# FluidInference/FluidAudio

Hardware: NVIDIA H100
Metric: audio-hours/s (higher is better)
Workload: dtype f32

## Files before the change

fluidaudio_b200/csrc/mel_core.cuh:

```cuda
#pragma once

#include "fa_common.cuh"
#include <math.h>
#include <stdint.h>

namespace fa {
namespace mel {

constexpr int kNfft = 512;
constexpr int kHalf = 256;
constexpr int kBins = 257;
constexpr int kFftPad = 304;
constexpr int kTileFrames = 16;
constexpr int kPairStride = 524;
FA_HD int pow_pos(int bin) { return bin ^ ((bin >> 4) & 3); }

struct alignas(8) cpx {
    float x, y;
};

struct alignas(8) f32x2 {
    float a, b;
};

#if defined(__CUDA_ARCH__)
__device__ __forceinline__ float2 as_f2(f32x2 v) { return make_float2(v.a, v.b); }
__device__ __forceinline__ f32x2 as_v(float2 v) {
    f32x2 r;
    r.a = v.x;
    r.b = v.y;
    return r;
}
#endif

FA_HD double vadd(double x, double y) { return x + y; }
FA_HD double vsub(double x, double y) { return x - y; }
FA_HD double vneg(double x) { return -x; }
FA_HD double vmul_s(double x, double s) { return x * s; }
FA_HD double vfma_s(double a, double s, double c) { return a * s + c; }
FA_HD double vfnma_s(double a, double s, double c) { return c - a * s; }

FA_HD f32x2 vneg(f32x2 x) {
    f32x2 r;
    r.a = -x.a;
    r.b = -x.b;
    return r;
}
#if defined(__CUDA_ARCH__)
__device__ __forceinline__ f32x2 vadd(f32x2 x, f32x2 y) { return as_v(fadd2_rn(as_f2(x), as_f2(y))); }
__device__ __forceinline__ f32x2 vsub(f32x2 x, f32x2 y) { return as_v(fadd2_rn(as_f2(x), as_f2(vneg(y)))); }
__device__ __forceinline__ f32x2 vmul_s(f32x2 x, float s) { return as_v(fmul2_rn(as_f2(x), make_float2(s, s))); }
__device__ __forceinline__ f32x2 vfma_s(f32x2 a, float s, f32x2 c) {
    return as_v(ffma2_rn(as_f2(a), make_float2(s, s), as_f2(c)));
}
__device__ __forceinline__ f32x2 vfnma_s(f32x2 a, float s, f32x2 c) {
    return as_v(ffma2_rn(as_f2(vneg(a)), make_float2(s, s), as_f2(c)));
}
#else
inline f32x2 vadd(f32x2 x, f32x2 y) { return f32x2{x.a + y.a, x.b + y.b}; }
inline f32x2 vsub(f32x2 x, f32x2 y) { return f32x2{x.a - y.a, x.b - y.b}; }
inline f32x2 vmul_s(f32x2 x, float s) { return f32x2{x.a * s, x.b * s}; }
inline f32x2 vfma_s(f32x2 a, float s, f32x2 c) { return f32x2{fmaf(a.a, s, c.a), fmaf(a.b, s, c.b)}; }
inline f32x2 vfnma_s(f32x2 a, float s, f32x2 c) { return f32x2{fmaf(-a.a, s, c.a), fmaf(-a.b, s, c.b)}; }
#endif

template <typename V>
struct vtraits;
template <>
struct vtraits<double> {
    typedef double scalar;
    static constexpr int kFrames = 1;
};
template <>
struct vtraits<f32x2> {
    typedef float scalar;
    static constexpr int kFrames = 2;
};

template <typename V>
struct alignas(16) cpxv {
    V x, y;
};
typedef cpxv<double> cpxd;
struct cpxs {
    float x, y;
};

struct LaneCommon {
    float win[16];
    uint32_t in_win;
    int a1, a2, k0;
    int k0s, kc0s;
};
template <typename V>
struct LaneTables;
template <>
struct LaneTables<double> : LaneCommon {
    cpxd w256;
    cpxd w32;
    cpxd wk0;
};
template <>
struct LaneTables<f32x2> : LaneCommon {
    cpxs tw1[8];
    cpxs tw2[8];
    cpxs wk[4];
};

FA_HD void lane_butterflies(int l, int &c1, int &c2) {
    if (l >= 8) {
        c1 = l;
        c2 = 8 * (8 - (l >> 3)) + (7 - (l & 7));
    } else if (l >= 4) {
        c1 = 32 + (l - 4);
        c2 = 39 - (l - 4);
    } else if (l >= 1) {
        c1 = l;
        c2 = 8 - l;
    } else {
        c1 = 0;
        c2 = 4;
    }
}

FA_HD cpxd unit_root(int k, int n) {
    const double a = -6.283185307179586476925286766559 * (double)k / (double)n;
    cpxd r;
    r.x = cos(a);
    r.y = sin(a);
    return r;
}
FA_HD cpxs unit_root_f(int k, int n) {
    const cpxd d = unit_root(k, n);
    cpxs r;
    r.x = (float)d.x;
    r.y = (float)d.y;
    return r;
}

FA_HD void load_lane_common(int l, const float *win_tab, const uint8_t *in_tab, LaneCommon &T) {
    T.in_win = 0;
#pragma unroll
    for (int r = 0; r < 8; ++r) {
        const int j = 2 * (l + 32 * r);
        T.win[2 * r] = win_tab[j];
        T.win[2 * r + 1] = win_tab[j + 1];
        if (in_tab[j]) T.in_win |= 1u << (2 * r);
        if (in_tab[j + 1]) T.in_win |= 1u << (2 * r + 1);
    }
    int c1, c2;
    lane_butterflies(l, c1, c2);
    T.a1 = 9 * (c1 >> 3) + (c1 & 7);
    T.a2 = 9 * (c2 >> 3) + (c2 & 7);
    T.k0 = (c1 >> 3) + 8 * (c1 & 7);
    T.k0s = pow_pos(T.k0);
    T.kc0s = pow_pos(kHalf - T.k0);
}
FA_HD void load_lane_tables(int l, const float *win_tab, const uint8_t *in_tab, LaneTables<double> &T) {
    load_lane_common(l, win_tab, in_tab, T);
    T.w256 = unit_root(l, 256);
    T.w32 = unit_root(l & 3, 32);
    T.wk0 = unit_root(T.k0, 512);
}
FA_HD void load_lane_tables(int l, const float *win_tab, const uint8_t *in_tab, LaneTables<f32x2> &T) {
    load_lane_common(l, win_tab, in_tab, T);
#pragma unroll
    for (int q = 0; q < 8; ++q) {
        T.tw1[q] = unit_root_f((l * q) & 255, 256);
        T.tw2[q] = unit_root_f(((l & 3) * q) & 31, 32);
    }
#pragma unroll
    for (int k2 = 0; k2 < 4; ++k2) T.wk[k2] = unit_root_f(T.k0 + 64 * k2, 512);
}

FA_HD cpxd cmul(cpxd a, cpxd b) {
    cpxd r;
    r.x = a.x * b.x - a.y * b.y;
    r.y = a.x * b.y + a.y * b.x;
    return r;
}

template <typename V>
FA_HD void dft4(V &r0, V &i0, V &r1, V &i1, V &r2, V &i2, V &r3, V &i3) {
    const V ar = vadd(r0, r2), ai = vadd(i0, i2);
    const V br = vsub(r0, r2), bi = vsub(i0, i2);
    const V cr = vadd(r1, r3), ci = vadd(i1, i3);
    const V dr = vsub(r1, r3), di = vsub(i1, i3);
    r0 = vadd(ar, cr);
    i0 = vadd(ai, ci);
    r2 = vsub(ar, cr);
    i2 = vsub(ai, ci);
    r1 = vadd(br, di);
    i1 = vsub(bi, dr);
    r3 = vsub(br, di);
    i3 = vadd(bi, dr);
}

template <typename V>
FA_HD void dft8(V (&re)[8], V (&im)[8]) {
    typedef typename vtraits<V>::scalar S;
    const S kS = (S)0.70710678118654752440;
    V er0 = vadd(re[0], re[4]), ei0 = vadd(im[0], im[4]);
    V er1 = vadd(re[1], re[5]), ei1 = vadd(im[1], im[5]);
    V er2 = vadd(re[2], re[6]), ei2 = vadd(im[2], im[6]);
    V er3 = vadd(re[3], re[7]), ei3 = vadd(im[3], im[7]);
    V or0 = vsub(re[0], re[4]), oi0 = vsub(im[0], im[4]);
    const V xr1 = vsub(re[1], re[5]), xi1 = vsub(im[1], im[5]);
    const V xr2 = vsub(re[2], re[6]), xi2 = vsub(im[2], im[6]);
    const V xr3 = vsub(re[3], re[7]), xi3 = vsub(im[3], im[7]);
    V or1 = vmul_s(vadd(xr1, xi1), kS), oi1 = vmul_s(vsub(xi1, xr1), kS);
    V or2 = xi2, oi2 = vneg(xr2);
    V or3 = vmul_s(vsub(xi3, xr3), kS), oi3 = vmul_s(vadd(xr3, xi3), (S)(-kS));
    dft4(er0, ei0, er1, ei1, er2, ei2, er3, ei3);
    dft4(or0, oi0, or1, oi1, or2, oi2, or3, oi3);
    re[0] = er0; im[0] = ei0;
    re[2] = er1; im[2] = ei1;
    re[4] = er2; im[4] = ei2;
    re[6] = er3; im[6] = ei3;
    re[1] = or0; im[1] = oi0;
    re[3] = or1; im[3] = oi1;
    re[5] = or2; im[5] = oi2;
    re[7] = or3; im[7] = oi3;
}

template <typename Emit>
FA_HD void twiddle_emit(double (&re)[8], double (&im)[8], cpxd root, Emit emit) {
    cpxd p[8];
    p[1] = root;
    p[2] = cmul(root, root);
    p[3] = cmul(p[2], root);
    p[4] = cmul(p[2], p[2]);
    p[5] = cmul(p[4], root);
    p[6] = cmul(p[4], p[2]);
    p[7] = cmul(p[4], p[3]);
    cpxd v;
    v.x = re[0];
    v.y = im[0];
    emit(0, v);
#pragma unroll
    for (int q = 1; q < 8; ++q) {
        v.x = re[q] * p[q].x - im[q] * p[q].y;
        v.y = re[q] * p[q].y + im[q] * p[q].x;
        emit(q, v);
    }
}
template <typename Emit>
FA_HD void twiddle_emit(f32x2 (&re)[8], f32x2 (&im)[8], const cpxs (&tw)[8], Emit emit) {
    cpxv<f32x2> v;
    v.x = re[0];
    v.y = im[0];
    emit(0, v);
#pragma unroll
    for (int q = 1; q < 8; ++q) {
        v.x = vfnma_s(im[q], tw[q].y, vmul_s(re[q], tw[q].x));
        v.y = vfma_s(im[q], tw[q].x, vmul_s(re[q], tw[q].y));
        emit(q, v);
    }
}
FA_HD void twiddle_pass1(int l, double (&re)[8], double (&im)[8], const LaneTables<double> &T, cpxd *buf) {
    twiddle_emit(re, im, T.w256, [&](int q, cpxd v) { buf[l + 36 * q] = v; });
}
FA_HD void twiddle_pass1(int l, f32x2 (&re)[8], f32x2 (&im)[8], const LaneTables<f32x2> &T, cpxv<f32x2> *buf) {
    twiddle_emit(re, im, T.tw1, [&](int q, cpxv<f32x2> v) { buf[l + 36 * q] = v; });
}
FA_HD void twiddle_pass2(int base, double (&re)[8], double (&im)[8], const LaneTables<double> &T, cpxd *buf) {
    twiddle_emit(re, im, T.w32, [&](int q2, cpxd v) { buf[base + q2] = v; });
}
FA_HD void twiddle_pass2(int base, f32x2 (&re)[8], f32x2 (&im)[8], const LaneTables<f32x2> &T, cpxv<f32x2> *buf) {
    twiddle_emit(re, im, T.tw2, [&](int q2, cpxv<f32x2> v) { buf[base + q2] = v; });
}

FA_HD void widen(float a, float b, float, float, double &re, double &im) {
    re = (double)a;
    im = (double)b;
}
FA_HD void widen(float a, float b, float a2, float b2, f32x2 &re, f32x2 &im) {
    re.a = a;
    re.b = a2;
    im.a = b;
    im.b = b2;
}

template <bool kMidFull, typename V>
FA_HD void pass1(int l, const float *pf, int hop, const LaneTables<V> &T, cpxv<V> *buf) {
    V re[8], im[8];
#pragma unroll
    for (int r = 0; r < 8; ++r) {
        const int j = 2 * (l + 32 * r);
#if defined(__CUDA_ARCH__)
        const float2 v = *reinterpret_cast<const float2 *>(pf + j);
        float2 u = v;
        if (vtraits<V>::kFrames == 2) u = *reinterpret_cast<const float2 *>(pf + hop + j);
#else
        const cpx v = *reinterpret_cast<const cpx *>(pf + j);
        cpx u = v;
        if (vtraits<V>::kFrames == 2) u = *reinterpret_cast<const cpx *>(pf + hop + j);
#endif
        float a = T.win[2 * r] * v.x, b = T.win[2 * r + 1] * v.y;
        float a2 = T.win[2 * r] * u.x, b2 = T.win[2 * r + 1] * u.y;
        if (!kMidFull || r == 0 || r == 7) {
            const bool ia = (T.in_win >> (2 * r)) & 1u, ib = (T.in_win >> (2 * r + 1)) & 1u;
            a = ia ? a : 0.0f;
            b = ib ? b : 0.0f;
            a2 = ia ? a2 : 0.0f;
            b2 = ib ? b2 : 0.0f;
        }
        widen(a, b, a2, b2, re[r], im[r]);
    }
    dft8(re, im);
    twiddle_pass1(l, re, im, T, buf);
}

template <typename V>
FA_HD void pass2_load(int l, const cpxv<V> *buf, V (&re)[8], V (&im)[8]) {
    const int base = 36 * (l >> 2) + (l & 3);
#pragma unroll
    for (int r = 0; r < 8; ++r) {
        const cpxv<V> v = buf[base + 4 * r];
        re[r] = v.x;
        im[r] = v.y;
    }
}
template <typename V>
FA_HD void pass2_store(int l, const LaneTables<V> &T, V (&re)[8], V (&im)[8], cpxv<V> *buf) {
    dft8(re, im);
    const int base = 74 * (l & 3) + 9 * (l >> 2);
    twiddle_pass2(base, re, im, T, buf);
}

FA_HD void pair_power(double zbx, double zby, double zcx, double zcy, double wx, double wy, float *prow, int ib, int ic) {
    const double sr = zbx + zcx, si = zby - zcy;
    const double dr = zby + zcy, di = zcx - zbx;
    const double tr = wx * dr - wy * di, ti = wx * di + wy * dr;
    const float xr = (float)(sr + tr), xi = (float)(si + ti);
    const float yr = (float)(sr - tr), yi = (float)(si - ti);
#if defined(__CUDA_ARCH__)
    prow[2 * ib] = __fadd_rn(__fmul_rn(xr, xr), __fmul_rn(xi, xi));
    prow[2 * ic] = __fadd_rn(__fmul_rn(yr, yr), __fmul_rn(yi, yi));
#else
    const float a = xr * xr, b = xi * xi, c = yr * yr, d = yi * yi;
    prow[2 * ib] = a + b;
    prow[2 * ic] = c + d;
#endif
}
FA_HD void pair_power(f32x2 zbx, f32x2 zby, f32x2 zcx, f32x2 zcy, float wx, float wy, float *prow, int ib, int ic) {
    const f32x2 sr = vadd(zbx, zcx), si = vsub(zby, zcy);
    const f32x2 dr = vadd(zby, zcy), di = vsub(zcx, zbx);
    const f32x2 tr = vfnma_s(di, wy, vmul_s(dr, wx)), ti = vfma_s(dr, wy, vmul_s(di, wx));
    const f32x2 xr = vadd(sr, tr), xi = vadd(si, ti);
    const f32x2 yr = vsub(sr, tr), yi = vsub(si, ti);
#if defined(__CUDA_ARCH__)
    const float2 pb = ffma2_rn(as_f2(xr), as_f2(xr), fmul2_rn(as_f2(xi), as_f2(xi)));
    const float2 pc = ffma2_rn(as_f2(yr), as_f2(yr), fmul2_rn(as_f2(yi), as_f2(yi)));
    *reinterpret_cast<float2 *>(prow + 2 * ib) = pb;
    *reinterpret_cast<float2 *>(prow + 2 * ic) = pc;
#else
    prow[2 * ib] = fmaf(xr.a, xr.a, xi.a * xi.a);
    prow[2 * ic] = fmaf(yr.a, yr.a, yi.a * yi.a);
    prow[2 * ib + 1] = fmaf(xr.b, xr.b, xi.b * xi.b);
    prow[2 * ic + 1] = fmaf(yr.b, yr.b, yi.b * yi.b);
#endif
}

FA_HD void recombination_roots(const LaneTables<double> &T, double (&wx)[4], double (&wy)[4]) {
    const double hh = 0.70710678118654752440;
    wx[0] = T.wk0.x;
    wy[0] = T.wk0.y;
    wx[1] = hh * (wx[0] + wy[0]);
    wy[1] = hh * (wy[0] - wx[0]);
    wx[2] = wy[0];
    wy[2] = -wx[0];
    wx[3] = wy[1];
    wy[3] = -wx[1];
}
FA_HD void recombination_roots(const LaneTables<f32x2> &T, float (&wx)[4], float (&wy)[4]) {
#pragma unroll
    for (int k = 0; k < 4; ++k) {
        wx[k] = T.wk[k].x;
        wy[k] = T.wk[k].y;
    }
}

template <typename V>
FA_HD void pass3_post(int l, const cpxv<V> *buf, const LaneTables<V> &T, float *prow) {
    typedef typename vtraits<V>::scalar S;
    V ar[4], ai[4], br[4], bi[4];
#pragma unroll
    for (int h = 0; h < 4; ++h) {
        const cpxv<V> u = buf[T.a1 + 74 * h], v = buf[T.a2 + 74 * h];
        ar[h] = u.x;
        ai[h] = u.y;
        br[h] = v.x;
        bi[h] = v.y;
    }
    dft4(ar[0], ai[0], ar[1], ai[1], ar[2], ai[2], ar[3], ai[3]);
    dft4(br[0], bi[0], br[1], bi[1], br[2], bi[2], br[3], bi[3]);
    const bool z = l == 0;
    const S c1 = (S)0.92387953251128675613, s1 = (S)0.38268343236508977173;
    S wx[4], wy[4];
    recombination_roots(T, wx, wy);
    pair_power(ar[0], ai[0], z ? ar[0] : br[3], z ? ai[0] : bi[3], wx[0], wy[0], prow, T.k0s, T.kc0s);
    pair_power(ar[1], ai[1], z ? ar[3] : br[2], z ? ai[3] : bi[2], wx[1], wy[1], prow, T.k0s + 64, T.kc0s - 64);
    pair_power(ar[2], ai[2], z ? ar[2] : br[1], z ? ai[2] : bi[1], wx[2], wy[2], prow, T.k0s + 128, T.kc0s - 128);
    const int b3 = z ? pow_pos(32) : T.k0s + 192, c3 = z ? pow_pos(224) : T.kc0s - 192;
    pair_power(z ? br[0] : ar[3], z ? bi[0] : ai[3], z ? br[3] : br[0], z ? bi[3] : bi[0], z ? c1 : wx[3],
               z ? (S)(-s1) : wy[3], prow, b3, c3);
    if (z) {
        pair_power(br[1], bi[1], br[2], bi[2], s1, (S)(-c1), prow, pow_pos(96), pow_pos(160));
    }
}

FA_HD float mel_dot(const float *prow, const float *w, int lo, int hi) {
    float acc = 0.0f;
    const float *p = prow + lo;
    const int n = hi - lo;
    for (int b = 0; b < n; ++b) {
        const float t = w[b] * p[b];
        acc = acc + t;
    }
    return acc;
}
#if defined(__CUDACC__)
__device__ __forceinline__ float2 mel_dot_pairs(const float4 *p4, const float4 *w4, int nq) {
    float2 acc = make_float2(0.0f, 0.0f);
#pragma unroll 1
    for (int b = 0; b < nq; ++b) {
        const float4 x01 = p4[2 * b], x23 = p4[2 * b + 1], c = w4[b];
        acc = ffma2_rn(make_float2(x01.x, x01.y), make_float2(c.x, c.x), acc);
        acc = ffma2_rn(make_float2(x01.z, x01.w), make_float2(c.y, c.y), acc);
        acc = ffma2_rn(make_float2(x23.x, x23.y), make_float2(c.z, c.z), acc);
        acc = ffma2_rn(make_float2(x23.z, x23.w), make_float2(c.w, c.w), acc);
    }
    return acc;
}
__device__ __forceinline__ float mel_dot_quads(const float4 *p4, const float4 *w4, int nq) {
    float acc = 0.0f;
#pragma unroll 1
    for (int b = 0; b < nq; ++b) {
        const float4 x = p4[b], c = w4[b];
        acc = fmaf(c.x, x.x, acc);
        acc = fmaf(c.y, x.y, acc);
        acc = fmaf(c.z, x.z, acc);
        acc = fmaf(c.w, x.w, acc);
    }
    return acc;
}
#endif

FA_HD float log_value(float v, float floor_, int clamped, int normal_floor = 0) {
    const float x = clamped ? (floor_ >= v ? floor_ : v) : v + floor_;
#if defined(__CUDA_ARCH__)
    float l;
    if (normal_floor) asm("lg2.approx.ftz.f32 %0, %1;" : "=f"(l) : "f"(x));
    else l = __log2f(x);
    return l * 0.693147180559945309417f;
#else
    (void)normal_floor;
    return logf(x);
#endif
}

FA_HD float preemph_first(float x0, float last, float a) {
#if defined(__CUDA_ARCH__)
    return __fsub_rn(x0, __fmul_rn(a, last));
#else
    const float t = a * last;
    return x0 - t;
#endif
}
FA_HD float preemph_rest(float x, float xprev, float a) { return fmaf(xprev, -a, x); }

}
}
```

fluidaudio_b200/csrc/mel_kernels.cu:

```cuda
#include "mel_core.cuh"
#include "mel_plan.h"

#include <cuda_runtime.h>
#include <algorithm>
#include <cmath>
#include <cstdio>
#include <cstdlib>
#include <cstring>
#include <limits>
#include <vector>

namespace fa {
namespace mel {

__device__ __forceinline__ uint32_t smem_u32(const void *p) { return (uint32_t)__cvta_generic_to_shared(p); }

__device__ __forceinline__ void mbar_init(uint64_t *bar, uint32_t count) {
    asm volatile("mbarrier.init.shared::cta.b64 [%0], %1;" ::"r"(smem_u32(bar)), "r"(count));
}
__device__ __forceinline__ void mbar_expect_tx(uint64_t *bar, uint32_t bytes) {
    asm volatile("mbarrier.arrive.expect_tx.shared::cta.b64 _, [%0], %1;" ::"r"(smem_u32(bar)), "r"(bytes) : "memory");
}
__device__ __forceinline__ void mbar_arrive(uint64_t *bar) {
    asm volatile("mbarrier.arrive.shared::cta.b64 _, [%0];" ::"r"(smem_u32(bar)) : "memory");
}
__device__ __forceinline__ bool mbar_try_wait(uint64_t *bar, uint32_t parity) {
    uint32_t ok;
    asm volatile(
        "{\n\t"
        ".reg .pred p;\n\t"
        "mbarrier.try_wait.parity.shared::cta.b64 p, [%1], %2;\n\t"
        "selp.u32 %0, 1, 0, p;\n\t"
        "}"
        : "=r"(ok)
        : "r"(smem_u32(bar)), "r"(parity)
        : "memory");
    return ok != 0;
}
__device__ __forceinline__ void mbar_wait(uint64_t *bar, uint32_t parity) {
    while (!mbar_try_wait(bar, parity)) {
    }
}
__device__ __forceinline__ void bulk_g2s(void *dst, const void *src, uint32_t bytes, uint64_t *bar) {
    asm volatile("cp.async.bulk.shared::cluster.global.mbarrier::complete_tx::bytes [%0], [%1], %2, [%3];" ::"r"(
                     smem_u32(dst)),
                 "l"(src), "r"(bytes), "r"(smem_u32(bar))
                 : "memory");
}
__device__ __forceinline__ void fence_proxy_async() { asm volatile("fence.proxy.async.shared::cta;" ::: "memory"); }

struct TileGeom {
    int unit;
    long long f0;
    int nf;
    long long a0;
    long long base;
    long long gs, ge;
};

__device__ __forceinline__ const MelUnit &unit_at(const MelLaunch &P, int idx) { return P.inline_unit ? P.unit0 : P.units[idx]; }

__device__ __forceinline__ TileGeom tile_geom(const MelLaunch &P, int tile) {
    int lo = 0, hi = P.inline_unit ? 0 : P.num_units - 1;
    while (lo < hi) {
        const int mid = (lo + hi + 1) >> 1;
        if (P.units[mid].tile_begin <= tile) lo = mid; else hi = mid - 1;
    }
    const MelUnit &u = P.inline_unit ? P.unit0 : P.units[lo];
    TileGeom g;
    g.unit = lo;
    g.f0 = u.frame_begin + (long long)kTileFrames * (tile - u.tile_begin);
    const long long rem = u.frame_begin + u.frame_count - g.f0;
    g.nf = rem < kTileFrames ? (int)rem : kTileFrames;
    g.a0 = g.f0 * P.hop - P.pad;
    const long long need0 = g.a0 - 1;
    g.base = (need0 >= 0) ? (need0 & ~3LL) : -(((-need0) + 3) & ~3LL);
    long long ge = (g.a0 + P.pt_len + 3) & ~3LL;
    const long long n4 = u.n & ~3LL;
    if (ge > n4) ge = n4;
    g.gs = g.base < 0 ? 0 : g.base;
    g.ge = ge;
    if (!P.use_tma) g.ge = g.gs;
    return g;
}

struct TileInfo {
    TileGeom g;
    long long audio_off, n, out_off, out_stride;
    float last;
    int pad_;
};
__device__ __forceinline__ void make_tile_info(const MelLaunch &P, int tile, TileInfo &ti) {
    ti.g = tile_geom(P, tile);
    const MelUnit &u = unit_at(P, ti.g.unit);
    ti.audio_off = u.audio_off;
    ti.n = u.n;
    ti.out_off = u.out_off;
    ti.out_stride = u.out_stride;
    ti.last = u.last;
}

template <int kWarps, typename V, int kLayout>
__global__ void __launch_bounds__(kWarps * 32, 2) mel512_kernel(const MelLaunch P) {
    constexpr int kF = vtraits<V>::kFrames;
    extern __shared__ __align__(128) unsigned char smem[];
    float *raw0 = reinterpret_cast<float *>(smem);
    float *raw1 = raw0 + P.raw_cap;
    float *ptile = raw1 + P.raw_cap;
    cpxv<V> *fftbuf = reinterpret_cast<cpxv<V> *>(ptile + P.pt_cap);
    float *power = reinterpret_cast<float *>(fftbuf + kWarps * kFftPad);
    float *otile = power + (kTileFrames / 2) * kPairStride;
    const int ot_stride = P.ot_stride;
    float *fbw = otile + kTileFrames * ot_stride;
    int4 *fbmeta = reinterpret_cast<int4 *>(fbw + P.fb_cap);
    uint64_t *bars = reinterpret_cast<uint64_t *>(fbmeta + P.n_slots);
    TileInfo *tinfo = reinterpret_cast<TileInfo *>(bars + 2);

    const int tid = threadIdx.x, lane = tid & 31, warp = tid >> 5;

    if (tid == 0) {
        mbar_init(&bars[0], 1);
        mbar_init(&bars[1], 1);
        asm volatile("fence.mbarrier_init.release.cluster;" ::: "memory");
    }
    for (int i = tid; i < P.fb_nnz; i += kWarps * 32) fbw[i] = P.fb_w[i];
    for (int i = tid; i < P.n_slots; i += kWarps * 32) fbmeta[i] = P.fb_slots[i];
    for (int i = tid; i < (kTileFrames / 2) * kPairStride; i += kWarps * 32) power[i] = 0.0f;
    const LaneTables<V> T = reinterpret_cast<const LaneTables<V> *>(P.lane_tab)[lane];
    __syncthreads();

    cpxv<V> *buf = fftbuf + warp * kFftPad;

    auto issue = [&](int tile, int buf, TileInfo &slot) {
        make_tile_info(P, tile, slot);
        const TileGeom &g = slot.g;
        float *dst = buf ? raw1 : raw0;
        if (g.ge > g.gs) {
            const uint32_t bytes = (uint32_t)((g.ge - g.gs) * 4);
            mbar_expect_tx(&bars[buf], bytes);
            bulk_g2s(dst + (g.gs - g.base), P.audio + slot.audio_off + g.gs, bytes, &bars[buf]);
        } else {
            mbar_arrive(&bars[buf]);
        }
    };

    auto preemphasize = [&](const TileInfo &u, const float *raw) {
        const TileGeom &g = u.g;
        const float a = P.preemph;
        const bool interior = g.a0 >= 1 && g.a0 - 1 >= g.gs && g.a0 + P.pt_len <= g.ge && g.a0 + P.pt_len <= u.n;
        if (interior) {
            const float *src = raw + (g.a0 - g.base);
            if (((g.a0 - g.base) & 3) == 0 && (P.pt_len & 3) == 0) {
                const float4 *s4 = reinterpret_cast<const float4 *>(src);
                float4 *d4 = reinterpret_cast<float4 *>(ptile);
                for (int q = tid; q < (P.pt_len >> 2); q += kWarps * 32) {
                    const float4 x = s4[q];
                    float4 y = x;
                    const float prev = src[4 * q - 1];
                    if (a != 0.0f) {
                        y.x = preemph_rest(x.x, prev, a);
                        y.y = preemph_rest(x.y, x.x, a);
                        y.z = preemph_rest(x.z, x.y, a);
                        y.w = preemph_rest(x.w, x.z, a);
                    }
                    d4[q] = y;
                }
            } else if (a == 0.0f) {
                for (int t = tid; t < P.pt_len; t += kWarps * 32) ptile[t] = src[t];
            } else {
                for (int t = tid; t < P.pt_len; t += kWarps * 32) ptile[t] = preemph_rest(src[t], src[t - 1], a);
            }
        } else {
            const float *gaudio = P.audio + u.audio_off;
            auto sample = [&](long long i) -> float {
                if (i >= g.gs && i < g.ge) return raw[i - g.base];
                if (i < 0) return u.last;
                return __ldg(gaudio + i);
            };
            for (int t = tid; t < P.pt_len; t += kWarps * 32) {
                const long long i = g.a0 + t;
                float v = 0.0f;
                if (i >= 0 && i < u.n) {
                    const float x = sample(i);
                    if (a == 0.0f) v = x;
                    else if (i == 0) v = preemph_first(x, u.last, a);
                    else v = preemph_rest(x, sample(i - 1), a);
                }
                ptile[t] = v;
            }
        }
    };
    auto copy_out = [&](float *dst, int total) {
        if (P.out_vec4) {
            float4 *d4 = reinterpret_cast<float4 *>(dst);
            for (int q = tid; q < (total >> 2); q += kWarps * 32) {
                const int e = 4 * q;
                const int row = (int)__umulhi((unsigned)e, P.inv_n_mels);
                d4[q] = *reinterpret_cast<const float4 *>(otile + e + 4 * row);
            }
        } else {
            const int row_pad = ot_stride - P.n_mels;
            for (int idx = tid; idx < total; idx += kWarps * 32) {
                const int fi = P.n_mels == 1 ? idx : (int)__umulhi((unsigned)idx, P.inv_n_mels);
                dst[idx] = otile[idx + fi * row_pad];
            }
        }
    };

    const int first = blockIdx.x, stride = gridDim.x;
    if (first >= P.total_tiles) return;
    if (tid == 0) {
        issue(first, 0, tinfo[0]);
        if (first + stride < P.total_tiles) issue(first + stride, 1, tinfo[1]);
    }
    __syncthreads();
    mbar_wait(&bars[0], 0);
    preemphasize(tinfo[0], raw0);
    __syncthreads();
    float *pending_dst = nullptr;
    int pending_total = 0;
    int it = 0, slot = 0;
    for (int tile = first; tile < P.total_tiles; tile += stride, ++it, slot = slot == 2 ? 0 : slot + 1) {
        const TileInfo &u = tinfo[slot];
        const int nf = u.g.nf;

        if (pending_dst) copy_out(pending_dst, pending_total);
        for (int fi = warp * kF; fi < nf; fi += kWarps * kF) {
            const float *pf = ptile + fi * P.hop;
            V re[8], im[8];
            if (P.mid_full) pass1<true>(lane, pf, P.hop, T, buf); else pass1<false>(lane, pf, P.hop, T, buf);
            __syncwarp();
            pass2_load(lane, buf, re, im);
            __syncwarp();
            pass2_store(lane, T, re, im, buf);
            __syncwarp();
            pass3_post(lane, buf, T, power + (fi >> 1) * kPairStride + (fi & 1));
            __syncwarp();
        }
        __syncthreads();

        const int next = tile + stride;
        const int slot1 = slot == 2 ? 0 : slot + 1, slot2 = slot1 == 2 ? 0 : slot1 + 1;
        if (tid == 0 && next + stride < P.total_tiles) {
            fence_proxy_async();
            issue(next + stride, it & 1, tinfo[slot2]);
        }
        {
            constexpr int kPairs = kTileFrames / 2, kGroup = 32 / kPairs;
            const int pl = lane % kPairs, mg = lane / kPairs;
            const float *prow = power + pl * kPairStride;
            float *orow = otile + (2 * pl) * ot_stride;
            float *gout = kLayout == 1 ? P.out + u.out_off + u.g.f0 + 2 * pl : nullptr;
            for (int slot = warp * kGroup + mg; slot < P.n_slots; slot += kWarps * kGroup) {
                const int4 md = fbmeta[slot];
                const float2 a2 = mel_dot_pairs(reinterpret_cast<const float4 *>(prow + 2 * md.x),
                                                reinterpret_cast<const float4 *>(fbw + md.z), md.y);
                const float v0 = log_value(a2.x, P.log_floor, P.log_clamped, P.log_normal),
                            v1 = log_value(a2.y, P.log_floor, P.log_clamped, P.log_normal);
                const int m = md.w;
                if (m < 0) continue;
                if (kLayout == 0) {
                    orow[m] = v0;
                    orow[ot_stride + m] = v1;
                } else {
                    float *g = gout + (long long)m * u.out_stride;
                    if (2 * pl < nf) g[0] = v0;
                    if (2 * pl + 1 < nf) g[1] = v1;
                }
            }
        }
        if (kLayout == 0) {
            pending_dst = P.out + u.out_off + u.g.f0 * P.n_mels;
            pending_total = nf * P.n_mels;
        }
        if (next < P.total_tiles) {
            const int nb = (it + 1) & 1;
            mbar_wait(&bars[nb], (uint32_t)((it + 1) >> 1) & 1u);
            preemphasize(tinfo[slot1], nb ? raw1 : raw0);
        }
        __syncthreads();
    }
    if (pending_dst) copy_out(pending_dst, pending_total);
}


struct GenericParams {
    int n_fft, log2n, bins, prow;
    const cpxd *tw;
    int warps;
};

__global__ void __launch_bounds__(256) mel_generic_kernel(const MelLaunch P, const GenericParams G) {
    extern __shared__ __align__(16) unsigned char smem[];
    cpxd *tw = reinterpret_cast<cpxd *>(smem);
    cpxd *fft = tw + G.n_fft / 2;
    float *power = reinterpret_cast<float *>(fft + (size_t)G.warps * G.n_fft);
    float *win = power + (size_t)G.warps * G.prow;
    const int tid = threadIdx.x, lane = tid & 31, warp = tid >> 5, nthreads = G.warps * 32;
    for (int i = tid; i < G.n_fft / 2; i += nthreads) tw[i] = G.tw[i];
    for (int i = tid; i < G.n_fft; i += nthreads) win[i] = P.in_tab[i] ? P.win_tab[i] : 0.0f;
    for (int i = tid; i < G.warps * G.prow; i += nthreads) power[i] = 0.0f;
    __syncthreads();
    cpxd *buf = fft + (size_t)warp * G.n_fft;
    float *prow = power + (size_t)warp * G.prow;
    const float a = P.preemph;
    for (int tile = blockIdx.x; tile < P.total_tiles; tile += gridDim.x) {
        const TileGeom g = tile_geom(P, tile);
        const MelUnit u = unit_at(P, g.unit);
        const float *x = P.audio + u.audio_off;
        for (int fi = warp; fi < g.nf; fi += G.warps) {
            const long long f = g.f0 + fi;
            const long long base = f * P.hop - P.pad;
            for (int j = lane; j < G.n_fft; j += 32) {
                const long long i = base + j;
                float v = 0.0f;
                if (i >= 0 && i < u.n && P.in_tab[j]) {
                    const float xi = __ldg(x + i);
                    if (a == 0.0f) v = xi;
                    else if (i == 0) v = preemph_first(xi, u.last, a);
                    else v = preemph_rest(xi, __ldg(x + i - 1), a);
                    v = __fmul_rn(v, win[j]);
                }
                cpxd z;
                z.x = (double)v;
                z.y = 0.0;
                buf[__brev((unsigned)j) >> (32 - G.log2n)] = z;
            }
            __syncwarp();
            for (int s = 0; s < G.log2n; ++s) {
                const int half = 1 << s, step = G.n_fft >> (s + 1);
                for (int t = lane; t < G.n_fft / 2; t += 32) {
                    const int j = t & (half - 1);
                    const int ia = ((t >> s) << (s + 1)) + j, ib = ia + half;
                    const cpxd w = tw[j * step], zb = buf[ib], za = buf[ia];
                    const double tr = zb.x * w.x - zb.y * w.y, ti = zb.x * w.y + zb.y * w.x;
                    cpxd o;
                    o.x = za.x - tr;
                    o.y = za.y - ti;
                    buf[ib] = o;
                    o.x = za.x + tr;
                    o.y = za.y + ti;
                    buf[ia] = o;
                }
                __syncwarp();
            }
            for (int b = lane; b < G.bins; b += 32) {
                const float xr = (float)buf[b].x, xi = (float)buf[b].y;
                prow[b] = 4.0f * __fadd_rn(__fmul_rn(xr, xr), __fmul_rn(xi, xi));
            }
            __syncwarp();
            for (int m = lane; m < P.n_mels; m += 32) {
                const int lo = P.fb_lo[m], nq = (P.fb_hi[m] - lo) >> 2;
                const float v = log_value(mel_dot_quads(reinterpret_cast<const float4 *>(prow + lo),
                                                        reinterpret_cast<const float4 *>(P.fb_w + P.fb_off[m]), nq),
                                          P.log_floor, P.log_clamped);
                if (P.layout == 0) P.out[u.out_off + f * P.n_mels + m] = v;
                else P.out[u.out_off + (long long)m * u.out_stride + f] = v;
            }
            __syncwarp();
        }
    }
}

static float swift_float_pi() {
    const uint32_t bits = 0x40490FDAu;
    float f;
    std::memcpy(&f, &bits, 4);
    return f;
}

void build_window(int length, bool periodic, std::vector<float> &w) {
    w.resize(length);
    const float divisor = periodic ? (float)length : (float)(length - 1);
    const float pi = swift_float_pi();
    for (int i = 0; i < length; ++i) {
        const float phase = 2.0f * pi * (float)i / divisor;
        w[i] = 0.5f * (1.0f - cosf(phase));
    }
}

void build_filterbank(int n_fft, int n_mels, int sample_rate, std::vector<float> &fb) {
    const int bins = n_fft / 2 + 1;
    const float f_sp = 200.0f / 3.0f, min_log_hz = 1000.0f;
    const float min_log_mel = min_log_hz / f_sp;
    const float log_step = logf(6.4f) / 27.0f;
    auto to_mel = [&](float hz) { return hz >= min_log_hz ? min_log_mel + logf(hz / min_log_hz) / log_step : hz / f_sp; };
    auto to_hz = [&](float mel) {
        return mel >= min_log_mel ? min_log_hz * expf(log_step * (mel - min_log_mel)) : f_sp * mel;
    };
    const float mel_lo = to_mel(0.0f), mel_hi = to_mel((float)sample_rate / 2.0f);
    std::vector<float> edge(n_mels + 2), freq(bins);
    for (int i = 0; i < n_mels + 2; ++i) edge[i] = to_hz(mel_lo + (float)i * (mel_hi - mel_lo) / (float)(n_mels + 1));
    for (int i = 0; i < bins; ++i) freq[i] = (float)i * (float)sample_rate / (float)n_fft;
    fb.assign((size_t)n_mels * bins, 0.0f);
    for (int m = 0; m < n_mels; ++m) {
        const float l = edge[m], c = edge[m + 1], r = edge[m + 2];
        const float norm = 2.0f / (r - l);
        for (int b = 0; b < bins; ++b) {
            const float f = freq[b];
            if (f >= l && f < c) fb[(size_t)m * bins + b] = norm * (f - l) / (c - l);
            else if (f >= c && f <= r) fb[(size_t)m * bins + b] = norm * (r - f) / (r - c);
        }
    }
}

static constexpr int kWarpsPerCta = 8;
static constexpr int kCtasPerSm = 2;

MelPlan::~MelPlan() { release(); }

void MelPlan::release() {
    auto fr = [](auto *&p) {
        if (p) cudaFree(p);
        p = nullptr;
    };
    for (int m = 0; m < 2; ++m) {
        fr(d_win_tab_mode[m]);
        fr(d_in_tab_mode[m]);
        fr(d_lane_tab[m][0]);
        fr(d_lane_tab[m][1]);
    }
    fr(d_fb_w);
    fr(d_fb_slots);
    fr(d_fb_lo);
    fr(d_fb_hi);
    fr(d_fb_off);
    fr(d_units);
    fr(d_audio);
    fr(d_out);
    fr(d_pcm);
    fr(d_rs_tab);
    fr(d_generic_tw);
    rs_in = rs_out = 0.0;
    d_units_bytes = h_units_bytes = d_audio_bytes = d_out_bytes = d_pcm_bytes = rs_tab_bytes = 0;
    if (h_units) cudaFreeHost(h_units);
    h_units = nullptr;
    if (units_uploaded) cudaEventDestroy(units_uploaded);
    units_uploaded = nullptr;
    units_in_flight = false;
    for (auto &s : streams)
        if (s) cudaStreamDestroy(s), s = nullptr;
    for (auto &e : events)
        if (e) cudaEventDestroy(e);
    events.clear();
    for (auto &e : timer)
        if (e) cudaEventDestroy(e), e = nullptr;
}

int MelPlan::init(const MelConfig &c) {
    cfg = c;
    if (cfg.pad_to < 1) cfg.pad_to = 1;
    if (cfg.n_mels <= 0 || cfg.hop_length <= 0 || cfg.win_length <= 0 || cfg.n_fft <= 0 || cfg.sample_rate <= 0) {
        fa::set_error("mel config: all sizes must be positive");
        return FA_INVALID_ARGUMENT;
    }
    const bool pow2 = cfg.n_fft >= 32 && cfg.n_fft <= 4096 && (cfg.n_fft & (cfg.n_fft - 1)) == 0;
    if (!pow2 || cfg.win_length > cfg.n_fft || cfg.n_mels > 512 || cfg.hop_length > 65536) {
        fa::set_error("mel config unsupported by the sm_90a kernels: need nFFT a power of two in 32..4096, win <= nFFT, "
                      "nMels <= 512 (got nFFT=%d hop=%d win=%d nMels=%d)",
                      cfg.n_fft, cfg.hop_length, cfg.win_length, cfg.n_mels);
        return FA_UNSUPPORTED;
    }
    generic = cfg.n_fft != kNfft || (cfg.hop_length & 1) || cfg.hop_length > 1024;
    const int n_fft = cfg.n_fft, bins = n_fft / 2 + 1;
    build_window(cfg.win_length, cfg.window_periodic != 0, window);
    build_filterbank(cfg.n_fft, cfg.n_mels, cfg.sample_rate, filterbank);

    std::vector<int> lo(cfg.n_mels), hi(cfg.n_mels), off(cfg.n_mels);
    fb_nnz = 0;
    for (int m = 0; m < cfg.n_mels; ++m) {
        int a = bins, b = 0;
        for (int k = 0; k < bins; ++k)
            if (filterbank[(size_t)m * bins + k] != 0.0f) {
                a = std::min(a, k);
                b = k + 1;
            }
        if (b == 0) a = 0;
        a &= ~3;
        b = (b + 3) & ~3;
        lo[m] = a;
        hi[m] = b;
        off[m] = fb_nnz;
        fb_nnz += b - a;
    }
    std::vector<int4> slots;
    {
        const int groups = (cfg.n_mels + 3) / 4;
        std::vector<int> cost(groups, 0), order(groups);
        for (int g = 0; g < groups; ++g) {
            for (int m = 4 * g; m < std::min(cfg.n_mels, 4 * g + 4); ++m) cost[g] = std::max(cost[g], (hi[m] - lo[m]) >> 2);
            order[g] = g;
        }
        std::stable_sort(order.begin(), order.end(), [&](int a, int b) { return cost[a] > cost[b]; });
        std::vector<std::vector<int>> mine(kWarpsPerCta);
        std::vector<long long> load(kWarpsPerCta, 0);
        load[0] = 24;
        if (const char *h = std::getenv("FA_MEL_ISSUE_HANDICAP")) load[0] = std::atoi(h);
        for (int g : order) {
            int best = 0;
            for (int wv = 1; wv < kWarpsPerCta; ++wv)
                if (load[wv] + 2 * (long long)mine[wv].size() < load[best] + 2 * (long long)mine[best].size()) best = wv;
            mine[best].push_back(g);
            load[best] += cost[g] + 4;
        }
        size_t iters = 0;
        for (auto &v : mine) iters = std::max(iters, v.size());
        slots.assign(iters * kWarpsPerCta * 4, make_int4(0, 0, 0, -1));
        for (int wv = 0; wv < kWarpsPerCta; ++wv)
            for (size_t it = 0; it < mine[wv].size(); ++it)
                for (int q = 0; q < 4; ++q) {
                    const int m = 4 * mine[wv][it] + q;
                    if (m < cfg.n_mels) slots[(it * kWarpsPerCta + wv) * 4 + q] = make_int4(lo[m], (hi[m] - lo[m]) >> 2, off[m], m);
                }
    }
    n_slots = (int)slots.size();

    int dev = 0;
    FA_CUDA_TRY(cudaGetDevice(&dev));
    cudaDeviceProp prop;
    const int st = sm90_device_props(dev, prop);
    if (st != FA_OK) return st;
    num_sms = prop.multiProcessorCount;

    if (!generic) {
        pt_len = (kTileFrames - 1) * cfg.hop_length + kNfft;
        pt_cap = (pt_len + 31) & ~31;
        raw_cap = (pt_len + 1 + 3 + 3 + 31) & ~31;
        fb_cap = (fb_nnz + 3) & ~3;
        smem_bytes = sizeof(float) * ((size_t)2 * raw_cap + pt_cap + 0 +
                                      (size_t)(kTileFrames / 2) * kPairStride + (size_t)kTileFrames * (cfg.n_mels + 4) + fb_cap) +
                     sizeof(cpxd) * (size_t)kWarpsPerCta * kFftPad + sizeof(int) * 4 * (size_t)n_slots + 8 +
                     2 * sizeof(uint64_t) + 3 * sizeof(TileInfo) + 16;
        if (smem_bytes > (size_t)prop.sharedMemPerBlockOptin) {
            generic = true;
            pt_len = pt_cap = raw_cap = fb_cap = 0;
        }
    }
    std::vector<float> w;
    w.reserve(fb_nnz);
    for (int m = 0; m < cfg.n_mels; ++m)
// ... 539 lines not shown
```

Baseline: 3069.

## Restructure f32 FFT as 16x16 radix-16 with shuffle-based mirror exchange

Replaces the packed two-frame f32x2 radix-8 FFT path with a scalar-float 16x16 decomposition in which each half-warp processes one frame using register DFT16 butterflies. The real-FFT mirror recombination now uses warp shuffles instead of an extra shared-memory round trip, which cuts the per-frame passes from four warp syncs to two. Per-lane tables are rebuilt for the new layout, and recombination roots are stashed once in shared memory. This gives up the paired FFMA2 instructions (not native on H100 anyway) in exchange for fewer shared-memory passes and syncs, at the cost of higher register pressure from the 16-element arrays.

```diff
diff --git a/fluidaudio_b200/csrc/mel_core.cuh b/fluidaudio_b200/csrc/mel_core.cuh
--- a/fluidaudio_b200/csrc/mel_core.cuh
+++ b/fluidaudio_b200/csrc/mel_core.cuh
@@ -23,16 +23,6 @@
     float a, b;
 };
 
-#if defined(__CUDA_ARCH__)
-__device__ __forceinline__ float2 as_f2(f32x2 v) { return make_float2(v.a, v.b); }
-__device__ __forceinline__ f32x2 as_v(float2 v) {
-    f32x2 r;
-    r.a = v.x;
-    r.b = v.y;
-    return r;
-}
-#endif
-
 FA_HD double vadd(double x, double y) { return x + y; }
 FA_HD double vsub(double x, double y) { return x - y; }
 FA_HD double vneg(double x) { return -x; }
@@ -40,28 +30,19 @@
 FA_HD double vfma_s(double a, double s, double c) { return a * s + c; }
 FA_HD double vfnma_s(double a, double s, double c) { return c - a * s; }
 
-FA_HD f32x2 vneg(f32x2 x) {
-    f32x2 r;
-    r.a = -x.a;
-    r.b = -x.b;
-    return r;
-}
+FA_HD float vneg(float x) { return -x; }
 #if defined(__CUDA_ARCH__)
-__device__ __forceinline__ f32x2 vadd(f32x2 x, f32x2 y) { return as_v(fadd2_rn(as_f2(x), as_f2(y))); }
-__device__ __forceinline__ f32x2 vsub(f32x2 x, f32x2 y) { return as_v(fadd2_rn(as_f2(x), as_f2(vneg(y)))); }
-__device__ __forceinline__ f32x2 vmul_s(f32x2 x, float s) { return as_v(fmul2_rn(as_f2(x), make_float2(s, s))); }
-__device__ __forceinline__ f32x2 vfma_s(f32x2 a, float s, f32x2 c) {
-    return as_v(ffma2_rn(as_f2(a), make_float2(s, s), as_f2(c)));
-}
-__device__ __forceinline__ f32x2 vfnma_s(f32x2 a, float s, f32x2 c) {
-    return as_v(ffma2_rn(as_f2(vneg(a)), make_float2(s, s), as_f2(c)));
-}
+__device__ __forceinline__ float vadd(float x, float y) { return __fadd_rn(x, y); }
+__device__ __forceinline__ float vsub(float x, float y) { return __fsub_rn(x, y); }
+__device__ __forceinline__ float vmul_s(float x, float s) { return __fmul_rn(x, s); }
+__device__ __forceinline__ float vfma_s(float a, float s, float c) { return __fmaf_rn(a, s, c); }
+__device__ __forceinline__ float vfnma_s(float a, float s, float c) { return __fmaf_rn(-a, s, c); }
 #else
-inline f32x2 vadd(f32x2 x, f32x2 y) { return f32x2{x.a + y.a, x.b + y.b}; }
-inline f32x2 vsub(f32x2 x, f32x2 y) { return f32x2{x.a - y.a, x.b - y.b}; }
-inline f32x2 vmul_s(f32x2 x, float s) { return f32x2{x.a * s, x.b * s}; }
-inline f32x2 vfma_s(f32x2 a, float s, f32x2 c) { return f32x2{fmaf(a.a, s, c.a), fmaf(a.b, s, c.b)}; }
-inline f32x2 vfnma_s(f32x2 a, float s, f32x2 c) { return f32x2{fmaf(-a.a, s, c.a), fmaf(-a.b, s, c.b)}; }
+inline float vadd(float x, float y) { return x + y; }
+inline float vsub(float x, float y) { return x - y; }
+inline float vmul_s(float x, float s) { return x * s; }
+inline float vfma_s(float a, float s, float c) { return fmaf(a, s, c); }
+inline float vfnma_s(float a, float s, float c) { return fmaf(-a, s, c); }
 #endif
 
 template <typename V>
@@ -101,9 +82,11 @@
     cpxd wk0;
 };
 template <>
-struct LaneTables<f32x2> : LaneCommon {
-    cpxs tw1[8];
-    cpxs tw2[8];
+struct LaneTables<f32x2> {
+    float win[32];
+    uint32_t in_win;
+    uint32_t xc;
+    cpxs tw[16];
     cpxs wk[4];
 };
 
@@ -163,14 +146,19 @@
     T.wk0 = unit_root(T.k0, 512);
 }
 FA_HD void load_lane_tables(int l, const float *win_tab, const uint8_t *in_tab, LaneTables<f32x2> &T) {
-    load_lane_common(l, win_tab, in_tab, T);
-#pragma unroll
-    for (int q = 0; q < 8; ++q) {
-        T.tw1[q] = unit_root_f((l * q) & 255, 256);
-        T.tw2[q] = unit_root_f(((l & 3) * q) & 31, 32);
-    }
-#pragma unroll
-    for (int k2 = 0; k2 < 4; ++k2) T.wk[k2] = unit_root_f(T.k0 + 64 * k2, 512);
+    const int c = l & 15;
+    T.in_win = 0;
+    for (int n = 0; n < 16; ++n) {
+        const int j = 2 * (c + 16 * n);
+        T.win[2 * n] = win_tab[j];
+        T.win[2 * n + 1] = win_tab[j + 1];
+        if (in_tab[j]) T.in_win |= 1u << (2 * n);
+        if (in_tab[j + 1]) T.in_win |= 1u << (2 * n + 1);
+    }
+    T.xc = 0;
+    for (int m = 0; m < 4; ++m) T.xc |= (uint32_t)(pow_pos(kHalf - c - 16 * m) - 16 * (15 - m)) << (8 * m);
+    for (int k = 0; k < 16; ++k) T.tw[k] = unit_root_f(c * k, 256);
+    for (int k = 0; k < 4; ++k) T.wk[k] = unit_root_f(c + 16 * k, 512);
 }
 
 FA_HD cpxd cmul(cpxd a, cpxd b) {
@@ -244,41 +232,16 @@
         emit(q, v);
     }
 }
-template <typename Emit>
-FA_HD void twiddle_emit(f32x2 (&re)[8], f32x2 (&im)[8], const cpxs (&tw)[8], Emit emit) {
-    cpxv<f32x2> v;
-    v.x = re[0];
-    v.y = im[0];
-    emit(0, v);
-#pragma unroll
-    for (int q = 1; q < 8; ++q) {
-        v.x = vfnma_s(im[q], tw[q].y, vmul_s(re[q], tw[q].x));
-        v.y = vfma_s(im[q], tw[q].x, vmul_s(re[q], tw[q].y));
-        emit(q, v);
-    }
-}
 FA_HD void twiddle_pass1(int l, double (&re)[8], double (&im)[8], const LaneTables<double> &T, cpxd *buf) {
     twiddle_emit(re, im, T.w256, [&](int q, cpxd v) { buf[l + 36 * q] = v; });
 }
-FA_HD void twiddle_pass1(int l, f32x2 (&re)[8], f32x2 (&im)[8], const LaneTables<f32x2> &T, cpxv<f32x2> *buf) {
-    twiddle_emit(re, im, T.tw1, [&](int q, cpxv<f32x2> v) { buf[l + 36 * q] = v; });
-}
 FA_HD void twiddle_pass2(int base, double (&re)[8], double (&im)[8], const LaneTables<double> &T, cpxd *buf) {
     twiddle_emit(re, im, T.w32, [&](int q2, cpxd v) { buf[base + q2] = v; });
-}
-FA_HD void twiddle_pass2(int base, f32x2 (&re)[8], f32x2 (&im)[8], const LaneTables<f32x2> &T, cpxv<f32x2> *buf) {
-    twiddle_emit(re, im, T.tw2, [&](int q2, cpxv<f32x2> v) { buf[base + q2] = v; });
 }
 
 FA_HD void widen(float a, float b, float, float, double &re, double &im) {
     re = (double)a;
     im = (double)b;
-}
-FA_HD void widen(float a, float b, float a2, float b2, f32x2 &re, f32x2 &im) {
-    re.a = a;
-    re.b = a2;
-    im.a = b;
-    im.b = b2;
 }
 
 template <bool kMidFull, typename V>
@@ -343,24 +306,6 @@
     prow[2 * ic] = c + d;
 #endif
 }
-FA_HD void pair_power(f32x2 zbx, f32x2 zby, f32x2 zcx, f32x2 zcy, float wx, float wy, float *prow, int ib, int ic) {
-    const f32x2 sr = vadd(zbx, zcx), si = vsub(zby, zcy);
-    const f32x2 dr = vadd(zby, zcy), di = vsub(zcx, zbx);
-    const f32x2 tr = vfnma_s(di, wy, vmul_s(dr, wx)), ti = vfma_s(dr, wy, vmul_s(di, wx));
-    const f32x2 xr = vadd(sr, tr), xi = vadd(si, ti);
-    const f32x2 yr = vsub(sr, tr), yi = vsub(si, ti);
-#if defined(__CUDA_ARCH__)
-    const float2 pb = ffma2_rn(as_f2(xr), as_f2(xr), fmul2_rn(as_f2(xi), as_f2(xi)));
-    const float2 pc = ffma2_rn(as_f2(yr), as_f2(yr), fmul2_rn(as_f2(yi), as_f2(yi)));
-    *reinterpret_cast<float2 *>(prow + 2 * ib) = pb;
-    *reinterpret_cast<float2 *>(prow + 2 * ic) = pc;
-#else
-    prow[2 * ib] = fmaf(xr.a, xr.a, xi.a * xi.a);
-    prow[2 * ic] = fmaf(yr.a, yr.a, yi.a * yi.a);
-    prow[2 * ib + 1] = fmaf(xr.b, xr.b, xi.b * xi.b);
-    prow[2 * ic + 1] = fmaf(yr.b, yr.b, yi.b * yi.b);
-#endif
-}
 
 FA_HD void recombination_roots(const LaneTables<double> &T, double (&wx)[4], double (&wy)[4]) {
     const double hh = 0.70710678118654752440;
@@ -372,13 +317,6 @@
     wy[2] = -wx[0];
     wx[3] = wy[1];
     wy[3] = -wx[1];
-}
-FA_HD void recombination_roots(const LaneTables<f32x2> &T, float (&wx)[4], float (&wy)[4]) {
-#pragma unroll
-    for (int k = 0; k < 4; ++k) {
-        wx[k] = T.wk[k].x;
-        wy[k] = T.wk[k].y;
-    }
 }
 
 template <typename V>
@@ -410,6 +348,225 @@
     }
 }
 
+constexpr int kF32Frame = 272;
+
+FA_HD void dft16(float (&re)[16], float (&im)[16]) {
+    const float kC = 0.92387953251128675613f, kS = 0.38268343236508977173f, kH = 0.70710678118654752440f;
+#pragma unroll
+    for (int a = 0; a < 4; ++a) dft4(re[a], im[a], re[a + 4], im[a + 4], re[a + 8], im[a + 8], re[a + 12], im[a + 12]);
+    auto rot = [](float &r, float &i, float c, float s) {
+        const float t = vfnma_s(i, s, vmul_s(r, c));
+        i = vfma_s(i, c, vmul_s(r, s));
+        r = t;
+    };
+    rot(re[5], im[5], kC, -kS);
+    rot(re[7], im[7], kS, -kC);
+    rot(re[13], im[13], kS, -kC);
+    rot(re[15], im[15], -kC, kS);
+    auto w8 = [&](int p) {
+        const float r = re[p], i = im[p];
+        re[p] = vmul_s(vadd(r, i), kH);
+        im[p] = vmul_s(vsub(i, r), kH);
+    };
+    auto w8_3 = [&](int p) {
+        const float r = re[p], i = im[p];
+        re[p] = vmul_s(vsub(i, r), kH);
+        im[p] = vmul_s(vadd(r, i), -kH);
+    };
+    w8(6);
+    w8(9);
+    w8_3(11);
+    w8_3(14);
+    {
+        const float r = re[10];
+        re[10] = im[10];
+        im[10] = vneg(r);
+    }
+#pragma unroll
+    for (int kb = 0; kb < 4; ++kb)
+        dft4(re[4 * kb], im[4 * kb], re[4 * kb + 1], im[4 * kb + 1], re[4 * kb + 2], im[4 * kb + 2], re[4 * kb + 3],
+             im[4 * kb + 3]);
+    float tr[16], ti[16];
+#pragma unroll
+    for (int p = 0; p < 16; ++p) {
+        tr[p] = re[p];
+        ti[p] = im[p];
+    }
+#pragma unroll
+    for (int kb = 0; kb < 4; ++kb)
+#pragma unroll
+        for (int ka = 0; ka < 4; ++ka) {
+            re[kb + 4 * ka] = tr[4 * kb + ka];
+            im[kb + 4 * ka] = ti[4 * kb + ka];
+        }
+}
+
+template <bool kMidFull>
+FA_HD void f32_pass1(int lane, const float *pf, int hop, const LaneTables<f32x2> &T, cpxv<f32x2> *buf) {
+    const int c = lane & 15, h = lane >> 4;
+    const float *p = pf + h * hop;
+    float re[16], im[16];
+#pragma unroll
+    for (int n = 0; n < 16; ++n) {
+        const cpx v = *reinterpret_cast<const cpx *>(p + 2 * (c + 16 * n));
+        float a = T.win[2 * n] * v.x, b = T.win[2 * n + 1] * v.y;
+        if (!kMidFull || n < 2 || n > 13) {
+            a = ((T.in_win >> (2 * n)) & 1u) ? a : 0.0f;
+            b = ((T.in_win >> (2 * n + 1)) & 1u) ? b : 0.0f;
+        }
+        re[n] = a;
+        im[n] = b;
+    }
+    dft16(re, im);
+    cpx *y = reinterpret_cast<cpx *>(buf) + h * kF32Frame + 17 * c;
+    y[0] = cpx{re[0], im[0]};
+#pragma unroll
+    for (int k = 1; k < 16; ++k)
+        y[k] = cpx{vfnma_s(im[k], T.tw[k].y, vmul_s(re[k], T.tw[k].x)), vfma_s(im[k], T.tw[k].x, vmul_s(re[k], T.tw[k].y))};
+}
+
+FA_HD void f32_pass2(int lane, const cpxv<f32x2> *buf, float (&re)[16], float (&im)[16]) {
+    const cpx *y = reinterpret_cast<const cpx *>(buf) + (lane >> 4) * kF32Frame + (lane & 15);
+#pragma unroll
+    for (int n = 0; n < 16; ++n) {
+        const cpx v = y[17 * n];
+        re[n] = v.x;
+        im[n] = v.y;
+    }
+    dft16(re, im);
+}
+
+FA_HD int f32_slot(int i) { return i < 4 ? i : i + 4; }
+FA_HD void f32_mirror_send(int lane, const float (&re)[16], const float (&im)[16], float (&out)[16]) {
+    const bool z = (lane & 15) == 0;
+#pragma unroll
+    for (int i = 0; i < 8; ++i) {
+        const int k = f32_slot(i);
+        out[2 * i] = z ? re[(16 - k) & 15] : re[15 - k];
+        out[2 * i + 1] = z ? im[(16 - k) & 15] : im[15 - k];
+    }
+}
+
+FA_HD float lane_exchange(float v, int src, int j, const float *stage) {
+#if defined(__CUDA_ARCH__)
+    (void)j;
+    (void)stage;
+    return __shfl_sync(0xffffffffu, v, src);
+#else
+    (void)v;
+    return stage[16 * src + j];
+#endif
+}
+
+FA_HD void f32_pair_power(float zbx, float zby, float zcx, float zcy, float wx, float wy, float *pb, float *pc) {
+    const float sr = vadd(zbx, zcx), si = vsub(zby, zcy);
+    const float dr = vadd(zby, zcy), di = vsub(zcx, zbx);
+    const float tr = vfnma_s(di, wy, vmul_s(dr, wx)), ti = vfma_s(dr, wy, vmul_s(di, wx));
+    const float xr = vadd(sr, tr), xi = vadd(si, ti);
+    const float yr = vsub(sr, tr), yi = vsub(si, ti);
+    *pb = vfma_s(xr, xr, vmul_s(xi, xi));
+    *pc = vfma_s(yr, yr, vmul_s(yi, yi));
+}
+
+struct alignas(16) cpxs2 {
+    cpxs a, b;
+};
+FA_HD void f32_stash_roots(int lane, const LaneTables<f32x2> &T, cpxv<f32x2> *buf) {
+    cpxs2 *rt = reinterpret_cast<cpxs2 *>(reinterpret_cast<cpx *>(buf) + 2 * kF32Frame);
+    if (lane < 16) {
+        rt[lane] = cpxs2{T.wk[0], T.wk[1]};
+        rt[16 + lane] = cpxs2{T.wk[2], T.wk[3]};
+    }
+}
+
+FA_HD void f32_post(int lane, const float (&re)[16], const float (&im)[16], const LaneTables<f32x2> &T,
+                    const cpxv<f32x2> *buf, float *prow, const float *stage) {
+    const int c = lane & 15, h = lane >> 4;
+    const int src = ((16 - c) & 15) | (lane & 16);
+    float out[16], mr[8], mi[8];
+    f32_mirror_send(lane, re, im, out);
+#pragma unroll
+    for (int i = 0; i < 8; ++i) {
+        mr[i] = lane_exchange(out[2 * i], src, 2 * i, stage);
+        mi[i] = lane_exchange(out[2 * i + 1], src, 2 * i + 1, stage);
+    }
+    const cpxs2 *rt = reinterpret_cast<const cpxs2 *>(reinterpret_cast<const cpx *>(buf) + 2 * kF32Frame);
+    const cpxs2 r01 = rt[c], r23 = rt[16 + c];
+    const cpxs wk[4] = {r01.a, r01.b, r23.a, r23.b};
+    float *row = prow + h;
+#pragma unroll
+    for (int i = 0; i < 8; ++i) {
+        const int k = f32_slot(i), m = k & 3;
+        const float wx = k < 4 ? wk[m].x : wk[m].y, wy = k < 4 ? wk[m].y : -wk[m].x;
+        const int xb = c ^ m, xc = (int)((T.xc >> (8 * m)) & 0xffu);
+        f32_pair_power(re[k], im[k], mr[i], mi[i], wx, wy, row + 2 * (16 * k + xb), row + 2 * (16 * (15 - k) + xc));
+    }
+    if (c == 0) {
+        const float kH = 0.70710678118654752440f;
+        f32_pair_power(re[4], im[4], re[12], im[12], kH, -kH, row + 2 * pow_pos(64), row + 2 * pow_pos(192));
+    }
+}
+
+#if !defined(__CUDACC__)
+inline float *f32_stage(cpxv<f32x2> *buf) { return reinterpret_cast<float *>(buf); }
+inline const float *f32_stage(const cpxv<f32x2> *buf) { return reinterpret_cast<const float *>(buf); }
+template <bool kMidFull>
+inline void pass1(int l, const float *pf, int hop, const LaneTables<f32x2> &T, cpxv<f32x2> *buf) {
+    f32_stash_roots(l, T, buf);
+    f32_pass1<kMidFull>(l, pf, hop, T, buf);
+}
+inline void pass2_load(int l, const cpxv<f32x2> *buf, f32x2 (&re)[8], f32x2 (&im)[8]) {
+    float r[16], i[16];
+    f32_pass2(l, buf, r, i);
+    for (int q = 0; q < 8; ++q) {
+        re[q] = f32x2{r[2 * q], r[2 * q + 1]};
+        im[q] = f32x2{i[2 * q], i[2 * q + 1]};
+    }
+}
+inline void f32_unpack(const f32x2 (&re)[8], const f32x2 (&im)[8], float (&r)[16], float (&i)[16]) {
+    for (int q = 0; q < 8; ++q) {
+        r[2 * q] = re[q].a;
+        r[2 * q + 1] = re[q].b;
+        i[2 * q] = im[q].a;
+        i[2 * q + 1] = im[q].b;
+    }
+}
+inline void pass2_store(int l, const LaneTables<f32x2> &, f32x2 (&re)[8], f32x2 (&im)[8], cpxv<f32x2> *buf) {
+    float r[16], i[16], out[16];
+    f32_unpack(re, im, r, i);
+    f32_mirror_send(l, r, i, out);
+    float *st = f32_stage(buf);
+    for (int j = 0; j < 16; ++j) st[16 * l + j] = out[j];
+    for (int s = 0; s < 8; ++s) {
+        st[512 + 16 * l + 2 * s] = r[f32_slot(s)];
+        st[512 + 16 * l + 2 * s + 1] = i[f32_slot(s)];
+    }
+    if ((l & 15) == 0) {
+        float *x = st + 1024 + 4 * (l >> 4);
+        x[0] = r[4];
+        x[1] = i[4];
+        x[2] = r[12];
+        x[3] = i[12];
+    }
+}
+inline void pass3_post(int l, const cpxv<f32x2> *buf, const LaneTables<f32x2> &T, float *prow) {
+    const float *st = f32_stage(buf);
+    float r[16] = {}, i[16] = {};
+    for (int s = 0; s < 8; ++s) {
+        r[f32_slot(s)] = st[512 + 16 * l + 2 * s];
+        i[f32_slot(s)] = st[512 + 16 * l + 2 * s + 1];
+    }
+    if ((l & 15) == 0) {
+        const float *x = st + 1024 + 4 * (l >> 4);
+        r[4] = x[0];
+        i[4] = x[1];
+        r[12] = x[2];
+        i[12] = x[3];
+    }
+    f32_post(l, r, i, T, buf, prow, st);
+}
+#endif
+
 FA_HD float mel_dot(const float *prow, const float *w, int lo, int hi) {
     float acc = 0.0f;
     const float *p = prow + lo;
diff --git a/fluidaudio_b200/csrc/mel_kernels.cu b/fluidaudio_b200/csrc/mel_kernels.cu
--- a/fluidaudio_b200/csrc/mel_kernels.cu
+++ b/fluidaudio_b200/csrc/mel_kernels.cu
@@ -130,6 +130,10 @@
     __syncthreads();
 
     cpxv<V> *buf = fftbuf + warp * kFftPad;
+    if constexpr (kF == 2) {
+        f32_stash_roots(lane, T, buf);
+        __syncwarp();
+    }
 
     auto issue = [&](int tile, int buf, TileInfo &slot) {
         make_tile_info(P, tile, slot);
@@ -227,15 +231,24 @@
         if (pending_dst) copy_out(pending_dst, pending_total);
         for (int fi = warp * kF; fi < nf; fi += kWarps * kF) {
             const float *pf = ptile + fi * P.hop;
-            V re[8], im[8];
-            if (P.mid_full) pass1<true>(lane, pf, P.hop, T, buf); else pass1<false>(lane, pf, P.hop, T, buf);
-            __syncwarp();
-            pass2_load(lane, buf, re, im);
-            __syncwarp();
-            pass2_store(lane, T, re, im, buf);
-            __syncwarp();
-            pass3_post(lane, buf, T, power + (fi >> 1) * kPairStride + (fi & 1));
-            __syncwarp();
+            if constexpr (kF == 2) {
+                float re[16], im[16];
+                if (P.mid_full) f32_pass1<true>(lane, pf, P.hop, T, buf); else f32_pass1<false>(lane, pf, P.hop, T, buf);
+                __syncwarp();
+                f32_pass2(lane, buf, re, im);
+                f32_post(lane, re, im, T, buf, power + (fi >> 1) * kPairStride, nullptr);
+                __syncwarp();
+            } else {
+                V re[8], im[8];
+                if (P.mid_full) pass1<true>(lane, pf, P.hop, T, buf); else pass1<false>(lane, pf, P.hop, T, buf);
+                __syncwarp();
+                pass2_load(lane, buf, re, im);
+                __syncwarp();
+                pass2_store(lane, T, re, im, buf);
+                __syncwarp();
+                pass3_post(lane, buf, T, power + (fi >> 1) * kPairStride + (fi & 1));
+                __syncwarp();
+            }
         }
         __syncthreads();
 
```

Result: faster. 3182 (median of 6 runs) (+3.7%).
